# fgnt/pb_chime5

Hardware: AMD Instinct MI355X
Metric: utterance-seconds enhanced/sec/GPU (24ch, 20 EM iters) (higher is better)
Workload: dtype f64

## Files before the change

### pb_chime5_amd/csrc/cacgmm.hip

```cpp
#include <algorithm>
#include <cmath>
#include <cstdlib>

#include "gss_internal.h"
#include "dense_wave.h"
#include "jacobi.h"

namespace {

#ifndef GSS_CHOL_PRIO
#define GSS_CHOL_PRIO 1
#endif
#ifndef GSS_ESTEP_PRIO
#define GSS_ESTEP_PRIO 1
#endif
constexpr int EM_TILE = 64;
constexpr int EM_TS = EM_TILE + 1;

enum { MODE_FIRST = 0, MODE_EM = 1, MODE_PREDICT = 2 };

__device__ __forceinline__ void set_progress_priority(int done, int total) {
    const int q4 = 4 * done / total;
    if (q4 <= 0) __builtin_amdgcn_s_setprio(3);
    else if (q4 == 1) __builtin_amdgcn_s_setprio(2);
// ... 823 lines not shown
        cplx t[NS][CB];
#pragma unroll
        for (int s = 0; s < NS; ++s)
#pragma unroll
            for (int j = 0; j < CB; ++j)
                t[s][j] = (lane + 64 * s < NE && c + j < cnt) ? src[(int64_t)(c + j) * K * NE + 64 * s]
                                                              : c_make(0.0, 0.0);
#pragma unroll
        for (int s = 0; s < NS; ++s)
#pragma unroll
            for (int j = 0; j < CB; ++j) vals[s] = c_add(vals[s], t[s][j]);
    }
#pragma unroll
    for (int s = 0; s < NS; ++s) {
        if (lane + 64 * s < NE) {
            vals[s].x = ((double)D * vals[s].x) / den;
            vals[s].y = ((double)D * vals[s].y) / den;
        }
    }
#pragma unroll
    for (int s = 0; s < NS; ++s) {
        const int p = ts.d12[s];
        if (p >= 0 && (p >> 8) == (p & 255)) {
            vals[s].y = 0.0;
            tr += vals[s].x;
        }
    }
    return wave_sum(tr);
}

template <int NS = COV_SLOTS>
__device__ inline void store_covariance(const cplx (&vals)[COV_SLOTS], int D, double shift,
                                        bool full, cplx *A, int ld, int lane, const TriSlots &ts) {
#pragma unroll
    for (int s = 0; s < NS; ++s) {
        const int p = ts.d12[s];
        if (p >= 0) {
            const int d1 = p >> 8, d2 = p & 255;
            cplx v = vals[s];
            if (d1 == d2) v.x -= shift;
            A[d2 * ld + d1] = c_conj(v);
            if (full) A[d1 * ld + d2] = v;
        }
    }
}

#ifdef GSS_CHOL_TRACE
__device__ long long g_chol_phase[4096 * 10];
extern "C" int gss_debug_chol_phase(long long *host, int entries) {
    return (int)hipMemcpyFromSymbol(host, HIP_SYMBOL(g_chol_phase), sizeof(long long) * 10 * entries);
}
#define CHOL_STAMP(slot)                                                              \
    do {                                                                              \
        const int wg_ = blockIdx.y * gridDim.x + blockIdx.x;                          \
        if (threadIdx.x == 0 && wg_ < 4096) g_chol_phase[wg_ * 10 + (slot)] = clock64(); \
    } while (0)
#else
#define CHOL_STAMP(slot)
#endif

template <int NR>
__device__ __forceinline__ bool class_update_chol(const cplx (&vals)[COV_SLOTS], int D, int K,
                                                  double eig_floor, cplx *A, int lane,
                                                  cplx *__restrict__ Mq_fk,
                                                  double *__restrict__ logdet_fk,
                                                  const TriSlots &ts,
                                                  const int *__restrict__ tab_cm = nullptr) {
    constexpr int ld = 8 * NR + 1;
    constexpr int NS = cov_slots_for(NR);
    double *dinv = reinterpret_cast<double *>(A + D * ld);
    double nb2 = 0.0;
#pragma unroll
    for (int s = 0; s < NS; ++s) {
        const int p = ts.d12[s];
        if (p >= 0)
            nb2 += ((p >> 8) == (p & 255) ? 1.0 : 2.0) * (vals[s].x * vals[s].x + vals[s].y * vals[s].y);
    }
    nb2 = wave_sum(nb2);
    CHOL_STAMP(4);
    store_covariance<NS>(vals, D, 0.0, true, A, ld, lane, ts);
    wave_sync();
    const int tx = lane & 7, ty = lane >> 3;
    cplx reg[NR][NR];
#pragma unroll
    for (int a = 0; a < NR; ++a)
#pragma unroll
        for (int b = 0; b < NR; ++b) {
            const int i = ty + 8 * a, kk = tx + 8 * b;
            reg[a][b] = (kk >= i && kk < D) ? A[i * ld + kk] : c_make(0.0, 0.0);
        }
    wave_sync();
    CHOL_STAMP(5);
    if (!chol_inverse_sweep<8, NR, true>(reg, D, A, ld, dinv, tx, ty)) return false;
    CHOL_STAMP(6);
#if GSS_CHOL_PRIO
    __builtin_amdgcn_s_setprio(0);
#endif
    double ldv = 0.0;
    for (int i = lane; i < D; i += 64) ldv -= 2.0 * log(dinv[i]);
    ldv = wave_sum(ldv);
    CHOL_STAMP(7);
    double ni2 = 0.0;
    const int NE = tri_count(D);
#pragma unroll
    for (int s = 0; s < NS; ++s) {
        const int p = tab_cm ? (lane + 64 * s < NE ? tab_cm[lane + 64 * s] : -1) : ts.d12[s];
        if (p < 0) continue;
        const int d1 = p >> 8, d2 = p & 255;
// ... 54 lines not shown
#pragma unroll
        for (int s = 0; s < 4; ++s) {
            const int idx = lane + 64 * s, i = idx / m, j = idx - i * m;
            if (idx < m * m) {
                V[idx] = basis[idx];
                if (i <= j) {
                    A[i * m + j] = rot[s];
                    A[j * m + i] = c_conj(rot[s]);
                }
            }
        }
        wave_sync();
    }
    jacobi_eigh_wave(A, V, m, lane, 20, warm);
    if (basis != nullptr) {
        for (int idx = lane; idx < m * m; idx += 64) basis[idx] = V[idx];
        if (lane == 0) *basis_valid = 1;
    }
    double lmax = -INFINITY;
    for (int i = lane; i < D; i += 64) lmax = fmax(lmax, A[i * m + i].x);
    lmax = wave_max(lmax);
    double ldv = 0.0;
    for (int i = lane; i < D; i += 64) {
        double l = A[i * m + i].x / fmax(lmax, GSS_TINY);
        l = fmax(l, eig_floor);
        lam[i] = 1.0 / l;
        ldv += log(l);
    }
    ldv = wave_sum(ldv);
    wave_sync();
#pragma unroll
    for (int s = 0; s < COV_SLOTS; ++s) {
        const int p = ts.d12[s];
        if (p < 0) continue;
        const int e = lane + 64 * s, d1 = p >> 8, d2 = p & 255;
        cplx v = c_make(0.0, 0.0);
        for (int j = 0; j < D; ++j) {
            const cplx a = V[d1 * m + j], b = V[d2 * m + j];
            const double il = lam[j];
            v.x += il * (a.x * b.x + a.y * b.y);
            v.y += il * (a.y * b.x - a.x * b.y);
        }
        if (d1 == d2) {
            v.y = 0.0;
        } else {
            v.x *= 2.0;
            v.y *= 2.0;
        }
        Mq_fk[(int64_t)e * K] = v;
    }
    if (lane == 0) *logdet_fk = ldv;
}

template <int NR>
__global__ __launch_bounds__(64) void em_chol_kernel(const cplx *__restrict__ Bp,
                                                     const double *__restrict__ Sg, int nch,
                                                     int sg_nch, int D,
                                                     int K, int64_t T, double eig_floor,
                                                     int force_eigh, cplx *__restrict__ Mq,
                                                     double *__restrict__ logdet,
                                                     double *__restrict__ pi,
                                                     int *__restrict__ need_eigh,
                                                     const int *__restrict__ tri_tab,
                                                     MsegPlan plan,
                                                     const int *__restrict__ zero_tiles, int ntile) {
    extern __shared__ __attribute__((aligned(16))) char smem[];
    const int NE = tri_count(D);
    cplx *A = reinterpret_cast<cplx *>(smem);
    const int k = blockIdx.x, f = blockIdx.y, lane = threadIdx.x;
    const bool clamped = frequency_has_zero_frames(zero_tiles, ntile, f, lane);
    const int cnt = plan.S > 0 ? mseg_count(plan, f) : nch;

    CHOL_STAMP(0);
#if GSS_CHOL_PRIO
    __builtin_amdgcn_s_setprio(3);
#endif
    const TriSlots ts = tri_slots_tab(tri_tab, NE, lane);
    const double sg = sum_gamma(Sg, sg_nch, K, k, f, lane);
    const double den = fmax(sg, GSS_TINY);
    if (lane == 0) pi[f * K + k] = sg / (double)T;
    CHOL_STAMP(1);
    CHOL_STAMP(2);
    cplx vals[COV_SLOTS];
    const double tr = reduce_covariance<cov_slots_for(NR)>(Bp, nch, cnt, D, K, k, f, den, vals, lane, ts);
    CHOL_STAMP(3);
#if GSS_CHOL_PRIO
    __builtin_amdgcn_s_setprio(2);
#endif
    bool fast = !force_eigh && !clamped && tr > 0.0 && isfinite(tr);
    if (fast)
        fast = class_update_chol<NR>(vals, D, K, eig_floor, A, lane, Mq + (int64_t)f * NE * K + k,
                                     logdet + f * K + k, ts, tri_tab + NE);
    if (lane == 0) need_eigh[f * K + k] = fast ? 0 : 1;
    CHOL_STAMP(9);
}

__global__ __launch_bounds__(64) void em_eigh_kernel(const cplx *__restrict__ Bp,
                                                     const double *__restrict__ Sg, int nch,
                                                     int sg_nch, int D,
                                                     int K, double eig_floor,
                                                     const int *__restrict__ need_eigh,
                                                     cplx *__restrict__ Mq,
                                                     double *__restrict__ logdet,
                                                     const int *__restrict__ tri_tab,
                                                     MsegPlan plan) {
    const int k = blockIdx.x, f = blockIdx.y, lane = threadIdx.x;
    if (!need_eigh[f * K + k]) return;
    const int cnt = plan.S > 0 ? mseg_count(plan, f) : nch;
    extern __shared__ __attribute__((aligned(16))) char smem[];
    const int NE = tri_count(D);
    const double sg = sum_gamma(Sg, sg_nch, K, k, f, lane);
    const double den = fmax(sg, GSS_TINY);
    const TriSlots ts = tri_slots_tab(tri_tab, NE, lane);
    cplx vals[COV_SLOTS];
    reduce_covariance(Bp, nch, cnt, D, K, k, f, den, vals, lane, ts);
    class_update_eigh(vals, D, K, eig_floor, reinterpret_cast<cplx *>(smem), lane,
                      Mq + (int64_t)f * NE * K + k, logdet + f * K + k, ts);
}

__device__ __forceinline__ double row16_sum(double v) {
    double s = v + dpp_shifted<0x111, 0xf, 0xf>(v);
    s += dpp_shifted<0x112, 0xf, 0xf>(v);
    s += dpp_shifted<0x113, 0xf, 0xf>(v);
    s += dpp_shifted<0x114, 0xf, 0xe>(s);
    s += dpp_shifted<0x118, 0xf, 0xc>(s);
    return s;
}

constexpr int OC_FRAMES = 256;

#ifndef GSS_EM4_PRIO
#define GSS_EM4_PRIO 1
#endif
#ifdef GSS_EM4_TRACE
__device__ long long g_em4_phase[1024 * 6];
extern "C" int gss_debug_em4_phase(long long *host, int entries) {
    return (int)hipMemcpyFromSymbol(host, HIP_SYMBOL(g_em4_phase), sizeof(long long) * 6 * entries);
}
#define EM4_T(var) const long long var = __builtin_readcyclecounter()
#define EM4_ADD(slot, d) em4_acc[slot] += (d)
#else
#define EM4_T(var)
#define EM4_ADD(slot, d)
#endif

struct OnchipArgs {
    cplx *basis;
    const cplx *Yn;
    const uint8_t *act;
    int64_t act_stride, act_fstride;
    const double *init;
    int64_t init_stride, init_fstride;
    int64_t T;
    int F, iterations, iterations_post, force_eigh;
    int unmasked;
    const int *zero_tiles;
    int ntile;
    int cold_eigh;
    double eig_floor;
    double *gamma;
};

__device__ __forceinline__ bool class_update4_lane(const double (&b)[16], double eig_floor,
                                                   double (&m)[16], double &logdet) {
    constexpr int D = 4;
    cplx a[D][D];
    double nb2 = 0.0, tr = 0.0;
    {
        int off = 0;
#pragma unroll
// ... 627 lines not shown
};
EmStrides em_strides(const EmBlockPlan &p, int F, int64_t T, int D) {
    EmStrides s{0, 0, 0};
    for (int b : {0, p.nblocks - 1}) {
        const int Fb = em_block_size(p, F, b);
        int cf;
        const int nch = em_chunks(Fb, T, D, &cf);
        const int wpb = estep_waves_per_block(Fb, T);
        s.nch = std::max(s.nch, nch);
        s.reg_nch = std::max(s.reg_nch, wpb * (int)((T + 64 * wpb - 1) / (64 * wpb)));
    }
    s.bp_nch = std::max(s.nch, mstep_maxseg_limit());
    return s;
}

}

int psd_partials_run(gss_ctx *ctx, const cplx *Y, int F, int64_t T, int D, const double *W2,
                     int nch, int chunk_frames, cplx *part, int S) {
    const size_t lds = wcov_lds_layout(D, 2).total;
    const wcov_fn_t fn = D <= 4 ? wcov_kernel<2, false, false, false, 1>
                         : D <= 12 ? wcov_kernel<2, false, false, false, 3>
                         : D <= 24 ? wcov_kernel<2, false, false, false, 6> : wcov_kernel<2, false, false>;
    GSS_TRY(raise_lds_limit(ctx, fn, lds));
    hipLaunchKernelGGL(fn, dim3(xcd_grid(nch, F), S), dim3(256), lds,
                       ctx->stream, Y, W2, F, T, D, tri_count(D), nch, chunk_frames, part, 2, 0,
                       MsegPlan{});
    GSS_LAUNCH_CHECK(ctx, "wcov_kernel");
    return GSS_OK;
}

int psd3_partials_run(gss_ctx *ctx, const cplx *Y, int F, int64_t T, int D, const double *W3,
                      int nch, int chunk_frames, cplx *part) {
    const size_t lds = wcov_lds_layout(D, 3).total;
    const wcov_fn_t fn = D <= 4 ? wcov_kernel<3, false, false, false, 1>
                         : D <= 12 ? wcov_kernel<3, false, false, false, 3>
                         : D <= 24 ? wcov_kernel<3, false, false, false, 6> : wcov_kernel<3, false, false>;
    GSS_TRY(raise_lds_limit(ctx, fn, lds));
    hipLaunchKernelGGL(fn, dim3(xcd_grid(nch, F)), dim3(256), lds, ctx->stream, Y, W3, F, T, D,
                       tri_count(D), nch, chunk_frames, part, 3, 0, MsegPlan{});
    GSS_LAUNCH_CHECK(ctx, "wcov_kernel");
    return GSS_OK;
}

struct EmWork {
    cplx *Mq;
    double *logdet, *pi, *W;
    cplx *Bp;
    double *Sg_lds;
    cplx *Yn;
    double *Sg_reg;
    int *need_eigh;
    int *zero_tiles;
    int *tri_tab;
    cplx *basis;
};
static EmWork em_blocks(Workspace &ws, int F, int64_t T, int D, int K, const EmStrides &st,
                        bool onchip) {
    const size_t NE = tri_count(D);
    EmWork k;
    k.Mq = ws.take<cplx>((size_t)F * NE * K, "cacgmm Mq");
    k.logdet = ws.take<double>((size_t)F * K, "cacgmm logdet");
    k.pi = ws.take<double>((size_t)F * K, "cacgmm pi");
    k.W = ws.take<double>((size_t)F * K * T, "cacgmm W");
    k.Bp = ws.take<cplx>((size_t)F * st.bp_nch * K * NE, "cacgmm Bp");
    k.Sg_lds = ws.take<double>((size_t)F * st.nch * K, "cacgmm Sg");
    k.Yn = ws.take<cplx>((size_t)F * D * T, "cacgmm Yn");
    k.Sg_reg = ws.take<double>((size_t)F * st.reg_nch * K, "cacgmm Sg (register form)");
    k.need_eigh = ws.take<int>((size_t)F * K, "cacgmm need_eigh");
    k.zero_tiles = ws.take<int>((size_t)F * ((T + EM_TILE - 1) / EM_TILE), "cacgmm zero_tiles");
    k.tri_tab = ws.take<int>(2 * NE, "cacgmm tri_tab");
    k.basis = onchip ? ws.take<cplx>((size_t)F * K * 16, "cacgmm basis") : nullptr;
    return k;
}

size_t cacgmm_workspace_bytes(int F, int64_t T, int D, int K, bool one_block) {
    const EmBlockPlan bp = one_block ? EmBlockPlan{F, 1, 1} : em_block_plan(F, T, D, K);
    Workspace ws;
    em_blocks(ws, F, T, D, K, em_strides(bp, F, T, D), true);
    return ws.bytes + 4096;
}

namespace {
struct EmBlock {
    EmArgs a;
    int F, f0;
    cplx *Mq, *Yn;
    int *need_eigh, *zero_tiles;
    double *Sg_lds, *Sg_reg;
    int nch_lds, reg_nch, bp_nch, sg_nch;
    hipStream_t stream;
};
struct StreamRestore {
    gss_ctx *ctx;
    hipStream_t s;
    ~StreamRestore() { ctx->stream = s; }
};
}

int cacgmm_run(gss_ctx *ctx, const cplx *Y, int F, int64_t T, int D, const EmGuide &guide, int K,
               int iterations, int iterations_post, double *gamma) {
    EmSchedule s;
    s.iterations = iterations;
    s.model_iterations = std::max(iterations_post - 1, 0);
    s.model_masked = false;
    s.predict_masked = iterations_post == 0;
    s.gamma = gamma;
    s.onchip_allowed = true;
    return cacgmm_schedule_run(ctx, Y, F, T, D, guide, K, s);
}

int cacgmm_schedule_run(gss_ctx *ctx, const cplx *Y, int F, int64_t T, int D, const EmGuide &guide,
                        int K, const EmSchedule &s) {
    const int NE = tri_count(D);
    const int iterations = s.iterations;
    double *const gamma = s.gamma;
    const bool reg = estep_reg_supported(D, K) && !gss_variant_set("estep_lds");
    const bool onchip = s.onchip_allowed && D == 4 && K >= 2 && K <= 6 && reg && iterations > 0 &&
                        !gss_variant_set("em_unfused") && !s.shared_prior;
    const EmBlockPlan bplan =
        onchip || s.shared_prior ? EmBlockPlan{F, 1, 1} : em_block_plan(F, T, D, K);
    const EmStrides st = em_strides(bplan, F, T, D);

    GSS_REQUIRE(ctx, !s.shared_prior || (!s.import_model && !s.export_model && !s.loglik),
                GSS_ERR_INVALID, "cacgmm: a model with a shared prior cannot leave the call");
    Workspace ws(ctx);
    const EmWork k = em_blocks(ws, F, T, D, K, st, onchip);
    EmPriorWork pw{};
    if (s.shared_prior) {
        pw = cacgmm_prior_alloc(ws, F, T, K, !s.prior);
        if (s.prior) pw.prior = s.prior;
    }
    GSS_TRY(ws.status("cacgmm"));
    cplx *const Mq = k.Mq, *const Bp = k.Bp, *const Yn = k.Yn;
    double *const logdet = k.logdet, *const pi = k.pi, *const W = k.W;
    double *const Sg_lds = k.Sg_lds, *const Sg_reg = k.Sg_reg;
    int *const need_eigh = k.need_eigh, *const zero_tiles = k.zero_tiles, *const tri_tab = k.tri_tab;
    const int ntile = (int)((T + EM_TILE - 1) / EM_TILE);
    GSS_REQUIRE(ctx, em_estep_lds(D, K) <= 160 * 1024 &&
                         wcov_lds_layout(D, std::min(K, 8)).total <= 160 * 1024,
                GSS_ERR_UNSUPPORTED, "cacgmm: D=%d K=%d LDS", D, K);
    const bool has_mask = guide.mask != nullptr;
    const uint8_t *const act = has_mask ? guide.mask : reinterpret_cast<const uint8_t *>(Yn);
    const int64_t act_stride = has_mask ? guide.mask_k_stride : 0;
    const int64_t act_fstride = has_mask ? guide.mask_f_stride : 0;
    const int m = D + (D & 1);
    const size_t eigh_lds = (sizeof(cplx) * 2 * m * m + sizeof(double) * m + 15) / 16 * 16;
    const int force_eigh = gss_variant_set("force_eigh");
    if (!onchip) {
        hipLaunchKernelGGL(tri_table_kernel, dim3(1), dim3(256), 0, ctx->stream, D, tri_tab);
        GSS_LAUNCH_CHECK(ctx, "tri_table_kernel");
    }
    GSS_REQUIRE(ctx, !onchip || (!s.import_model && !s.export_model && !s.loglik), GSS_ERR_INVALID,
                "cacgmm: the one-launch kernel keeps its model on the chip");
    if (s.import_model) GSS_TRY(cacgmm_model_import(ctx, *s.import_model, F, K, D, Mq, logdet, pi));

    auto make_block = [&](int f0, int Fb, hipStream_t stream, EmBlock *blk) -> int {
        EmBlock &b = *blk;
        b = EmBlock{};
        b.F = Fb;
        b.f0 = f0;
        b.stream = stream;
        EmArgs &a = b.a;
        a.Y = Y + (int64_t)f0 * T * D;
        a.act = act + (int64_t)f0 * act_fstride;
        a.act_stride = act_stride;
        a.act_fstride = act_fstride;
        a.init = guide.init ? guide.init + (int64_t)f0 * guide.init_f_stride : nullptr;
        a.init_stride = guide.init_k_stride;
        a.init_fstride = guide.init_f_stride;
        a.T = T;
        a.F = Fb;
        a.D = D;
        a.NE = NE;
        a.nch = em_chunks(Fb, T, D, &a.chunk_frames);
        GSS_TRY(mstep_plan(ctx, Fb, T, D, K, &a.mseg));
        b.bp_nch = a.mseg.S > 0 ? a.mseg.maxseg : a.nch;
        b.nch_lds = a.nch;
        const int wpb = estep_waves_per_block(Fb, T);
        b.reg_nch = wpb * (int)((T + 64 * wpb - 1) / (64 * wpb));
        GSS_REQUIRE(ctx, b.bp_nch <= st.bp_nch && b.nch_lds <= st.nch && b.reg_nch <= st.reg_nch,
                    GSS_ERR_INVALID, "cacgmm: block strides");
        b.Mq = Mq + (int64_t)f0 * NE * K;
        a.logdet = logdet + (int64_t)f0 * K;
        a.pi = pi + (int64_t)f0 * K;
        a.W = W + (int64_t)f0 * K * T;
        a.Bp = Bp + (int64_t)f0 * st.bp_nch * K * NE;
        b.Sg_lds = Sg_lds + (int64_t)f0 * st.nch * K;
        b.Sg_reg = Sg_reg + (int64_t)f0 * st.reg_nch * K;
        a.Sg = b.Sg_lds;
        a.gamma = gamma ? gamma + (int64_t)f0 * K * T : nullptr;
        b.Yn = Yn + (int64_t)f0 * D * T;
        b.need_eigh = need_eigh + (int64_t)f0 * K;
        b.zero_tiles = zero_tiles + (int64_t)f0 * ntile;
        b.sg_nch = b.nch_lds;
        return GSS_OK;
    };
    auto prepare = [&](EmBlock &b) -> int {
        GSS_PROF(ctx, "em_prepare");
        const size_t plds = sizeof(cplx) * (size_t)D * EM_TS + sizeof(double) * 4 * EM_TILE;
        const auto prep = D <= 4 ? em_prepare_kernel<1> : D <= 12 ? em_prepare_kernel<3>
                          : D <= 24 ? em_prepare_kernel<6> : em_prepare_kernel<8>;
        hipLaunchKernelGGL(prep,
                           dim3(xcd_grid((int)((T + EM_TILE - 1) / EM_TILE), b.F)), dim3(256), plds,
                           ctx->stream, b.a.Y, b.F, T, D, b.Yn, b.zero_tiles);
        GSS_LAUNCH_CHECK(ctx, "em_prepare_kernel");
        return GSS_OK;
    };
    auto estep = [&](EmBlock &b, int mode) -> int {
        EmArgs &a = b.a;
        if (s.shared_prior) {
            a.Sg = pw.Sg;
            const EmPriorArgs p{b.Yn, b.Mq, a.logdet, pw.prior, a.act, a.act_stride, a.act_fstride,
                                a.init, a.init_stride, a.init_fstride, a.W, pw.G, pw.Sg, a.gamma,
                                T, b.F, D, a.masked, a.aff_eps};
            return cacgmm_prior_estep_run(ctx, p, K, mode == MODE_FIRST ? EM_PRIOR_FIRST
                                                     : mode == MODE_EM  ? EM_PRIOR_FIT
                                                                        : EM_PRIOR_PREDICT);
        }
        if (reg && mode != MODE_FIRST) {
            a.Sg = b.Sg_reg;
            switch (D) {
                case 24: return launch_estep_reg_k<24>(ctx, K, mode, a, b.Mq, b.Yn, b.F);
                case 20: return launch_estep_reg_k<20>(ctx, K, mode, a, b.Mq, b.Yn, b.F);
                case 12: return launch_estep_reg_k<12>(ctx, K, mode, a, b.Mq, b.Yn, b.F);
                case 10: return launch_estep_reg_k<10>(ctx, K, mode, a, b.Mq, b.Yn, b.F);
                default: return launch_estep_reg_k<4>(ctx, K, mode, a, b.Mq, b.Yn, b.F);
            }
        }
        a.Sg = b.Sg_lds;
        return launch_estep_k(ctx, K, mode, a, b.Mq, b.F);
    };
    auto eig = [&](EmBlock &b) -> int {
        EmArgs &a = b.a;
        {
            GSS_PROF(ctx, "em_chol");
            const int nr = (D + 7) / 8;
            const size_t lds = sizeof(cplx) * (size_t)D * (8 * nr + 1) + sizeof(double) * D;
            auto kern = nr <= 1 ? em_chol_kernel<1> : nr == 2 ? em_chol_kernel<2>
                        : nr == 3 ? em_chol_kernel<3> : em_chol_kernel<4>;
            hipLaunchKernelGGL(kern, dim3(K, b.F), dim3(64), lds, ctx->stream, a.Bp, a.Sg, b.bp_nch,
                               b.sg_nch, D, K, T, 1e-10, force_eigh, b.Mq,
                               const_cast<double *>(a.logdet), const_cast<double *>(a.pi),
                               b.need_eigh, tri_tab, a.mseg, b.zero_tiles, ntile);
            GSS_LAUNCH_CHECK(ctx, "em_chol_kernel");
        }
        {
            GSS_PROF(ctx, "em_eigh");
            hipLaunchKernelGGL(em_eigh_kernel, dim3(K, b.F), dim3(64), eigh_lds, ctx->stream, a.Bp,
                               a.Sg, b.bp_nch, b.sg_nch, D, K, 1e-10, b.need_eigh, b.Mq,
                               const_cast<double *>(a.logdet), tri_tab, a.mseg);
            GSS_LAUNCH_CHECK(ctx, "em_eigh_kernel");
        }
        return GSS_OK;
    };

    if (onchip) {
        EmBlock b;
        GSS_TRY(make_block(0, F, ctx->stream, &b));
        GSS_TRY(prepare(b));
        OnchipArgs o{};
        o.basis = k.basis;
        o.Yn = Yn;
        o.act = act;
        o.act_stride = act_stride;
        o.act_fstride = act_fstride;
        o.init = guide.init;
        o.init_stride = guide.init_k_stride;
        o.init_fstride = guide.init_f_stride;
        o.unmasked = has_mask ? 0 : 1;
        o.T = T;
        o.F = F;
        o.iterations = iterations;
        o.iterations_post = s.predict_masked ? 0 : s.model_iterations + 1;
        o.force_eigh = force_eigh;
        o.zero_tiles = b.zero_tiles;
        o.ntile = ntile;
        o.cold_eigh = gss_variant_set("em4_cold_eigh");
        o.eig_floor = 1e-10;
        o.gamma = gamma;
        switch (K) {
            case 2: return launch_onchip4<2>(ctx, o);
            case 3: return launch_onchip4<3>(ctx, o);
            case 4: return launch_onchip4<4>(ctx, o);
            case 5: return launch_onchip4<5>(ctx, o);
            default: return launch_onchip4<6>(ctx, o);
        }
    }

    auto em_iteration = [&](EmBlock &b, bool first) -> int {
        GSS_TRY(estep(b, first ? MODE_FIRST : MODE_EM));
        b.sg_nch = s.shared_prior ? ntile : (reg && !first) ? b.reg_nch : b.nch_lds;
        if (s.shared_prior) {
            const bool one_table = guide.init ? guide.init_f_stride == 0 : guide.mask_f_stride == 0;
            GSS_TRY(cacgmm_prior_update_run(ctx, pw, first && one_table ? 1 : F, K, T));
        }
        GSS_TRY(launch_mstep_k(ctx, K, b.a, b.Yn, b.F));
        return eig(b);
    };

// ... 56 lines not shown
```

### pb_chime5_amd/csrc/gss_api.hip

```cpp
#include <cmath>
#include <cstdarg>
#include <cstdlib>
#include <cstring>
#include <mutex>

#include "gss_internal.h"

#define GSS_ENTER(ctx)                                   \
    if (!(ctx)) return GSS_ERR_INVALID;                  \
    GSS_HIP_CHECK((ctx), hipSetDevice((ctx)->device))
#define GSS_ENTER_VARIANTS(ctx) \
    GSS_ENTER(ctx);             \
    GSS_TRY(variant_refresh(ctx))
static int variant_refresh(gss_ctx *ctx);

#define GSS_STATUS_REF_CHANNEL 0
#define GSS_STATUS_WPE_ZERO_PIVOTS 2

static std::mutex g_error_lock;

int gss_fail(gss_ctx *ctx, int code, const char *fmt, ...) {
    char buf[1024];
    va_list ap;
    va_start(ap, fmt);
    vsnprintf(buf, sizeof(buf), fmt, ap);
    va_end(ap);
    if (ctx) {
        std::lock_guard<std::mutex> guard(g_error_lock);
        ctx->error = buf;
    }
    return code;
}

static thread_local std::string g_create_error;

namespace {
const char *const kVariantKeys[] = {
    "corr_ts", "corr_nw", "corr_blocked", "corr_p_tiles", "chol_diag_unfolded", "apply_ph",
    "apply_generic", "prof_detail", "corr_stg8", "corr_ksplit", "apply_gglobal", "wpe_halves",
    "em_wgs", "estep_wpb", "estep_lds", "mstep_prefetch_d", "mstep_tiled", "mstep_plan_min_d",
    "mstep_chunked", "mstep_slots", "force_eigh", "em_unfused", "em_l3_mb", "em_l3_fit_mb",
    "em_streams", "mstep_maxseg", "em4_cold_eigh", "mstep_generic",
    "wpe_online_mem"};
struct VariantTable {
    std::mutex lock;
    std::string text;
    bool parsed = false;
    std::map<std::string, int> values;
};
VariantTable &variant_table() {
    static VariantTable t;
    return t;
}
}

static int variant_refresh(gss_ctx *ctx) {
    const char *env = getenv("GSS_VARIANT");
    VariantTable &t = variant_table();
    std::lock_guard<std::mutex> guard(t.lock);
    if (t.parsed && t.text == (env ? env : "")) return GSS_OK;
    t.text = env ? env : "";
    t.parsed = true;
    t.values.clear();
    std::string unknown;
    size_t pos = 0;
    while (pos < t.text.size()) {
        size_t end = t.text.find_first_of(", ", pos);
        if (end == std::string::npos) end = t.text.size();
        const std::string tok = t.text.substr(pos, end - pos);
        pos = end + 1;
        if (tok.empty()) continue;
        const size_t eq = tok.find('=');
        const std::string name = tok.substr(0, eq);
        bool known = false;
        for (const char *k : kVariantKeys) known = known || name == k;
        if (!known) {
            unknown = name;
            continue;
        }
        t.values[name] = eq == std::string::npos ? 1 : atoi(tok.c_str() + eq + 1);
    }
    if (!unknown.empty()) {
        t.values.clear();
        t.parsed = false;
        return gss_fail(ctx, GSS_ERR_INVALID, "GSS_VARIANT names no switch '%s'", unknown.c_str());
    }
    return GSS_OK;
}

int gss_variant(const char *key, int dflt) {
    VariantTable &t = variant_table();
    std::lock_guard<std::mutex> guard(t.lock);
    const auto it = t.values.find(key);
    return it == t.values.end() ? dflt : it->second;
}
// ... 45 lines not shown
        g_create_error = "device_id out of range";
        return GSS_ERR_INVALID;
    }
    e = hipSetDevice(device_id);
    if (e != hipSuccess) {
        g_create_error = hipGetErrorString(e);
        return GSS_ERR_HIP;
    }
    gss_ctx *ctx = new gss_ctx();
    ctx->device = device_id;
    e = hipStreamCreateWithFlags(&ctx->own_stream, hipStreamNonBlocking);
    if (e != hipSuccess) {
        g_create_error = hipGetErrorString(e);
        delete ctx;
        return GSS_ERR_HIP;
    }
    ctx->stream = ctx->own_stream;
    e = hipHostMalloc(reinterpret_cast<void **>(&ctx->status_host), GSS_STATUS_BYTES,
                      hipHostMallocMapped);
    if (e == hipSuccess)
        e = hipHostGetDevicePointer(reinterpret_cast<void **>(&ctx->status_dev), ctx->status_host, 0);
    if (e != hipSuccess) {
        g_create_error = hipGetErrorString(e);
        (void)hipStreamDestroy(ctx->own_stream);
        delete ctx;
        return GSS_ERR_HIP;
    }
    ctx->status_host[GSS_STATUS_REF_CHANNEL] = INT32_MIN;
    ctx->status_host[GSS_STATUS_WPE_ZERO_PIVOTS] = 0;
    ctx->status_host[GSS_STATUS_SEGMENT_FALLBACKS] = 0;
    ctx->status_host[GSS_STATUS_LCMV_INTERFERER] = -1;
    ctx->status_host[GSS_STATUS_LCMV_FALLBACKS] = 0;
    ctx->status_host[GSS_STATUS_WPD_ZERO_PIVOTS] = 0;
    ctx->status_host[GSS_STATUS_ALIGN_MOVED] = 0;
    *out = ctx;
    return GSS_OK;
}

static void free_tables(gss_ctx *ctx) {
    if (ctx->win_analysis) (void)hipFree(ctx->win_analysis);
    if (ctx->win_synthesis) (void)hipFree(ctx->win_synthesis);
    if (ctx->twiddle) (void)hipFree(ctx->twiddle);
    ctx->win_analysis = ctx->win_synthesis = nullptr;
    ctx->twiddle = nullptr;
}

extern "C" int gss_destroy(gss_ctx *ctx) {
    if (!ctx) return GSS_OK;
    (void)hipSetDevice(ctx->device);
    (void)hipStreamSynchronize(ctx->stream);
    free_tables(ctx);
    if (ctx->arena) (void)hipFree(ctx->arena);
    if (ctx->wpe_tiles) (void)hipFree(ctx->wpe_tiles);
    if (ctx->status_host) (void)hipHostFree(ctx->status_host);
    for (auto &p : ctx->prof_pending) {
        (void)hipEventDestroy(p.start);
        (void)hipEventDestroy(p.stop);
    }
    for (auto ev : ctx->event_pool) (void)hipEventDestroy(ev);
    if (ctx->ev_fork) (void)hipEventDestroy(ctx->ev_fork);
    if (ctx->ev_join) (void)hipEventDestroy(ctx->ev_join);
    if (ctx->aux_stream) {
        (void)hipStreamSynchronize(ctx->aux_stream);
        (void)hipStreamDestroy(ctx->aux_stream);
    }
    if (ctx->own_stream) (void)hipStreamDestroy(ctx->own_stream);
    delete ctx;
    return GSS_OK;
}

int aux_stream_ready(gss_ctx *ctx) {
    if (!ctx->aux_stream)
        GSS_HIP_CHECK(ctx, hipStreamCreateWithFlags(&ctx->aux_stream, hipStreamNonBlocking));
    if (!ctx->ev_fork) GSS_HIP_CHECK(ctx, hipEventCreateWithFlags(&ctx->ev_fork, hipEventDisableTiming));
    if (!ctx->ev_join) GSS_HIP_CHECK(ctx, hipEventCreateWithFlags(&ctx->ev_join, hipEventDisableTiming));
    return GSS_OK;
}

extern "C" int gss_set_stream(gss_ctx *ctx, void *hip_stream) {
    GSS_ENTER(ctx);
    GSS_HIP_CHECK(ctx, hipStreamSynchronize(ctx->stream));
    ctx->stream = hip_stream ? reinterpret_cast<hipStream_t>(hip_stream) : ctx->own_stream;
    return GSS_OK;
}

extern "C" int gss_set_utterances_in_flight(gss_ctx *ctx, int n) {
    if (!ctx) return GSS_ERR_INVALID;
    GSS_REQUIRE(ctx, n >= 0, GSS_ERR_INVALID, "gss_set_utterances_in_flight: n=%d", n);
    ctx->utterances_in_flight = n;
    return GSS_OK;
}

extern "C" int gss_synchronize(gss_ctx *ctx) {
    if (!ctx) return GSS_ERR_INVALID;
    GSS_HIP_CHECK(ctx, hipSetDevice(ctx->device));
    GSS_HIP_CHECK(ctx, hipStreamSynchronize(ctx->stream));
    return GSS_OK;
}

extern "C" int gss_dev_malloc(gss_ctx *ctx, size_t bytes, void **dev_ptr) {
    if (!ctx || !dev_ptr) return GSS_ERR_INVALID;
    GSS_HIP_CHECK(ctx, hipSetDevice(ctx->device));
    *dev_ptr = nullptr;
    if (bytes == 0) bytes = 16;
    hipError_t e = hipMalloc(dev_ptr, bytes);
    if (e != hipSuccess)
// ... 154 lines not shown
            if (ctx->debug_violations++ == 0) {
                char text[256];
                snprintf(text, sizeof(text),
                         "the guard headroom of the workspace debug mode (%zu bytes) is used up at "
                         "block %d%s%s: no sizing bug of the call",
                         kDebugHeadroom, ctx->debug_blocks, tag ? " " : "", tag ? tag : "");
                ctx->debug_first = text;
            }
            return nullptr;
        }
        ctx->debug_guards.push_back({ctx->debug_blocks++, off, bytes, phys + bytes,
                                     guard_end - (phys + bytes), tag, false});
        ctx->debug_phys = guard_end;
        ctx->arena_off = off + bytes;
        if (ctx->arena_off > ctx->arena_peak) ctx->arena_peak = ctx->arena_off;
        return ctx->arena + phys;
    }
    if (off + bytes > ctx->arena_size) return nullptr;
    ctx->arena_off = off + bytes;
    if (ctx->arena_off > ctx->arena_peak) ctx->arena_peak = ctx->arena_off;
    return ctx->arena + off;
}

int arena_release_debug(gss_ctx *ctx, size_t mark) {
    GSS_TRY(debug_sync(ctx));
    while (!ctx->debug_guards.empty() &&
           ctx->debug_guards.back().logical_off + ctx->debug_guards.back().bytes > mark) {
        GSS_TRY(debug_check_guard(ctx, ctx->debug_guards.back()));
        ctx->debug_guards.pop_back();
    }
    ctx->arena_off = mark;
    ctx->debug_phys = ctx->debug_guards.empty()
                          ? 0
                          : ctx->debug_guards.back().guard_off + ctx->debug_guards.back().guard_bytes;
    GSS_HIP_CHECK(ctx, hipMemsetAsync(ctx->arena + ctx->debug_phys, ctx->debug_pattern,
                                      ctx->arena_size - ctx->debug_phys, ctx->stream));
    return GSS_OK;
}

extern "C" int gss_debug_workspace(gss_ctx *ctx, int pattern) {
    GSS_ENTER(ctx);
    GSS_REQUIRE(ctx, pattern >= -1 && pattern <= 255, GSS_ERR_INVALID,
                "gss_debug_workspace: pattern=%d (a byte, or -1 for off)", pattern);
    GSS_TRY(debug_sync(ctx));
    ctx->debug_pattern = pattern;
    ctx->debug_guards.clear();
    ctx->debug_blocks = 0;
    ctx->debug_phys = 0;
    ctx->debug_logical_size = 0;
    ctx->debug_violations = 0;
    ctx->debug_first.clear();
    ctx->arena_off = 0;
    ctx->wpe_tiles_key[0] = ctx->wpe_tiles_key[1] = ctx->wpe_tiles_key[2] = ctx->wpe_tiles_key[3] = -1;
    return GSS_OK;
}

extern "C" int gss_debug_workspace_report(gss_ctx *ctx, int64_t *violations, char *buf, int len,
                                          int guard_index, void **guard_dev) {
    GSS_ENTER(ctx);
    if (guard_dev) *guard_dev = nullptr;
    if (violations) *violations = 0;
    if (buf && len > 0) buf[0] = 0;
    GSS_REQUIRE(ctx, ctx->debug_pattern >= 0, GSS_ERR_INVALID,
                "gss_debug_workspace_report: the workspace debug mode is off");
    GSS_TRY(debug_check_live_guards(ctx));
    if (violations) *violations = ctx->debug_violations;
    if (buf && len > 0) snprintf(buf, (size_t)len, "%s", ctx->debug_first.c_str());
    if (guard_dev && guard_index >= 0 && (size_t)guard_index < ctx->debug_guards.size())
        *guard_dev = ctx->arena + ctx->debug_guards[guard_index].guard_off;
    return GSS_OK;
}

extern "C" size_t gss_workspace_bytes(gss_ctx *ctx) { return ctx ? ctx->arena_peak : 0; }

ProfScope::ProfScope(gss_ctx *c, const char *name) : ctx(c), active(c->profiling) {
    if (active && !c->prof_filter.empty() && c->prof_filter != name) active = false;
    if (!active) return;
    e.name = name;
    auto get = [&]() {
        hipEvent_t ev;
        if (!ctx->event_pool.empty()) {
            ev = ctx->event_pool.back();
            ctx->event_pool.pop_back();
        } else {
            (void)hipEventCreate(&ev);
        }
        return ev;
    };
    e.start = get();
    e.stop = get();
    (void)hipEventRecord(e.start, ctx->stream);
}

ProfScope::~ProfScope() {
    if (!active) return;
    (void)hipEventRecord(e.stop, ctx->stream);
    ctx->prof_pending.push_back(e);
}

static void prof_drain(gss_ctx *ctx) {
    (void)hipStreamSynchronize(ctx->stream);
    for (auto &p : ctx->prof_pending) {
        float ms = 0.f;
        if (hipEventElapsedTime(&ms, p.start, p.stop) == hipSuccess) {
            auto &acc = ctx->prof_acc[p.name];
            acc.first += 1;
// ... 1865 lines not shown
```

### pb_chime5_amd/csrc/gss_internal.h

```cpp
#pragma once
#include <hip/hip_runtime.h>

#include <cstdint>
#include <cstdio>
#include <map>
#include <string>
#include <vector>

#include "../../include/gss_hip.h"

typedef double2 cplx;

int gss_variant(const char *key, int dflt);
inline bool gss_variant_set(const char *key) { return gss_variant(key, 0) != 0; }

#if (defined(GSS_CORR_TRACE) || defined(GSS_WCOV_TRACE) || defined(GSS_EM4_TRACE) || \
     defined(GSS_CHOL_TRACE)) && !defined(GSS_EXPERIMENT_BUILD)
#error "trace instrumentation needs -DGSS_EXPERIMENT_BUILD=1 (tools/build_variant.sh)"
#endif

#define GSS_TINY 2.2250738585072014e-308

__device__ __forceinline__ cplx c_make(double r, double i) { return make_double2(r, i); }
__device__ __forceinline__ cplx c_add(cplx a, cplx b) { return make_double2(a.x + b.x, a.y + b.y); }
// ... 76 lines not shown
static inline unsigned xcd_grid(int nsub, int F) { return (unsigned)(nsub * ((F + 7) / 8 * 8)); }

__host__ __device__ __forceinline__ int tri_index(int d1, int d2, int D) {
    return d1 * D - (d1 * (d1 - 1)) / 2 + (d2 - d1);
}
__host__ __device__ __forceinline__ int tri_count(int D) { return D * (D + 1) / 2; }

struct ProfEntry {
    std::string name;
    hipEvent_t start, stop;
};

struct gss_ctx {
    int device = 0;
    hipStream_t own_stream = nullptr;
    hipStream_t stream = nullptr;
    hipStream_t aux_stream = nullptr;
    hipEvent_t ev_fork = nullptr, ev_join = nullptr;
    int utterances_in_flight = 0;
    std::string error;

    char *arena = nullptr;
    size_t arena_size = 0;
    size_t arena_off = 0;
    size_t arena_peak = 0;

    struct DebugGuard {
        int block;
        size_t logical_off, bytes;
        size_t guard_off, guard_bytes;
        const char *tag;
        bool reported;
    };
    int debug_pattern = -1;
    size_t debug_phys = 0;
    size_t debug_logical_size = 0;
    int debug_blocks = 0;
    std::vector<DebugGuard> debug_guards;
    int64_t debug_violations = 0;
    std::string debug_first;

    int stft_size = 0, stft_shift = 0;
    double *win_analysis = nullptr;
    double *win_synthesis = nullptr;
    cplx *twiddle = nullptr;

    int32_t *status_host = nullptr;
    int32_t *status_dev = nullptr;
    int last_targets = 0;
    int last_selected = 0;

    void *wpe_tiles = nullptr;
    int wpe_tiles_key[4] = {-1, -1, -1, -1};

    bool profiling = false;
    std::vector<ProfEntry> prof_pending;
    std::vector<hipEvent_t> event_pool;
    std::map<std::string, std::pair<long, double>> prof_acc;
    std::string prof_filter;
};

#define GSS_STATUS_SEGMENT_FALLBACKS 3
#define GSS_STATUS_LCMV_INTERFERER 4
#define GSS_STATUS_LCMV_FALLBACKS 5
#define GSS_STATUS_WPD_ZERO_PIVOTS 6
#define GSS_STATUS_ALIGN_MOVED 7
#define GSS_STATUS_MVDR_ONLINE_FALLBACKS 8
#define GSS_STATUS_CACGMM_ONLINE_FALLBACKS 9
#define GSS_STATUS_CACGMM_ONLINE_BAD_MODEL 10
#define GSS_STATUS_TARGETS 16
#define GSS_STATUS_CHANNELS 40
#define GSS_STATUS_BYTES (4 * (GSS_STATUS_CHANNELS + GSS_MAX_CHANNELS))
static_assert(GSS_STATUS_TARGETS + GSS_MAX_CLASSES + 1 <= GSS_STATUS_CHANNELS, "status words overlap");

int gss_fail(gss_ctx *ctx, int code, const char *fmt, ...);

#define GSS_HIP_CHECK(ctx, expr)                                                   \
    do {                                                                           \
        hipError_t _e = (expr);                                                    \
        if (_e != hipSuccess)                                                      \
            return gss_fail((ctx), GSS_ERR_HIP, "%s failed: %s (%s:%d)", #expr,    \
                            hipGetErrorString(_e), __FILE__, __LINE__);            \
    } while (0)

#define GSS_REQUIRE(ctx, cond, code, ...)                      \
    do {                                                       \
        if (!(cond)) return gss_fail((ctx), (code), __VA_ARGS__); \
    } while (0)

#define GSS_TRY(expr)              \
    do {                           \
        int _s = (expr);           \
        if (_s != GSS_OK) return _s; \
    } while (0)

int arena_reserve(gss_ctx *ctx, size_t bytes);
void arena_reset(gss_ctx *ctx);
void *arena_alloc(gss_ctx *ctx, size_t bytes, const char *tag);
int arena_release_debug(gss_ctx *ctx, size_t mark);
static inline int arena_release(gss_ctx *ctx, size_t mark) {
    if (ctx->debug_pattern >= 0) return arena_release_debug(ctx, mark);
    ctx->arena_off = mark;
    return GSS_OK;
}
static inline size_t align_up(size_t v, size_t a = 256) { return (v + a - 1) / a * a; }

// ... 230 lines not shown
```

Baseline: 1095.

## Fold eigh fallback into chol kernel, pack two waves per block, cache tri table

The Cholesky M-step kernel now packs two matrices per 128-thread workgroup, one per wave, over a flattened grid. Flagged matrices get the eigendecomposition fallback inside the same kernel after a block barrier, which removes the separate em_eigh launch per EM iteration by default. The triangle index table moves into the context and is rebuilt only when D changes, so the per-run tri_table_kernel launch goes away. The cost is a serialized fallback loop with __syncthreads and larger LDS per block, which may lower occupancy.

```diff
diff --git a/pb_chime5_amd/csrc/cacgmm.hip b/pb_chime5_amd/csrc/cacgmm.hip
--- a/pb_chime5_amd/csrc/cacgmm.hip
+++ b/pb_chime5_amd/csrc/cacgmm.hip
@@ -899,8 +899,8 @@
 }
 #define CHOL_STAMP(slot)                                                              \
     do {                                                                              \
-        const int wg_ = blockIdx.y * gridDim.x + blockIdx.x;                          \
-        if (threadIdx.x == 0 && wg_ < 4096) g_chol_phase[wg_ * 10 + (slot)] = clock64(); \
+        const int wg_ = blockIdx.x * (blockDim.x >> 6) + (threadIdx.x >> 6);    \
+        if ((threadIdx.x & 63) == 0 && wg_ < 4096) g_chol_phase[wg_ * 10 + (slot)] = clock64(); \
     } while (0)
 #else
 #define CHOL_STAMP(slot)
@@ -1061,47 +1061,97 @@
     if (lane == 0) *logdet_fk = ldv;
 }
 
+__device__ __forceinline__ void class_redo_eigh(const cplx *__restrict__ Bp,
+                                                const double *__restrict__ Sg, int nch, int sg_nch,
+                                                int D, int K, int k, int f, double eig_floor,
+                                                cplx *__restrict__ Mq, double *__restrict__ logdet,
+                                                const int *__restrict__ tri_tab, const MsegPlan &plan,
+                                                char *smem, int lane) {
+    const int cnt = plan.S > 0 ? mseg_count(plan, f) : nch;
+    const int NE = tri_count(D);
+    const double sg = sum_gamma(Sg, sg_nch, K, k, f, lane);
+    const double den = fmax(sg, GSS_TINY);
+    const TriSlots ts = tri_slots_tab(tri_tab, NE, lane);
+    cplx vals[COV_SLOTS];
+    reduce_covariance(Bp, nch, cnt, D, K, k, f, den, vals, lane, ts);
+    class_update_eigh(vals, D, K, eig_floor, reinterpret_cast<cplx *>(smem), lane,
+                      Mq + (int64_t)f * NE * K + k, logdet + f * K + k, ts);
+}
+
+__host__ __device__ constexpr size_t em_chol_wave_lds(int D, int NR) {
+    return (sizeof(cplx) * (size_t)D * (8 * NR + 1) + sizeof(double) * D + 15) / 16 * 16;
+}
+
 template <int NR>
-__global__ __launch_bounds__(64) void em_chol_kernel(const cplx *__restrict__ Bp,
-                                                     const double *__restrict__ Sg, int nch,
-                                                     int sg_nch, int D,
-                                                     int K, int64_t T, double eig_floor,
-                                                     int force_eigh, cplx *__restrict__ Mq,
-                                                     double *__restrict__ logdet,
-                                                     double *__restrict__ pi,
-                                                     int *__restrict__ need_eigh,
-                                                     const int *__restrict__ tri_tab,
-                                                     MsegPlan plan,
-                                                     const int *__restrict__ zero_tiles, int ntile) {
+__global__ __launch_bounds__(128) void em_chol_kernel(const cplx *__restrict__ Bp,
+                                                      const double *__restrict__ Sg, int nch,
+                                                      int sg_nch, int D,
+                                                      int K, int64_t T, double eig_floor,
+                                                      int force_eigh, cplx *__restrict__ Mq,
+                                                      double *__restrict__ logdet,
+                                                      double *__restrict__ pi,
+                                                      int *__restrict__ need_eigh,
+                                                      const int *__restrict__ tri_tab,
+                                                      MsegPlan plan,
+                                                      const int *__restrict__ zero_tiles, int ntile,
+                                                      int nmat, int redo_eigh, int flag_off) {
     extern __shared__ __attribute__((aligned(16))) char smem[];
     const int NE = tri_count(D);
-    cplx *A = reinterpret_cast<cplx *>(smem);
-    const int k = blockIdx.x, f = blockIdx.y, lane = threadIdx.x;
-    const bool clamped = frequency_has_zero_frames(zero_tiles, ntile, f, lane);
-    const int cnt = plan.S > 0 ? mseg_count(plan, f) : nch;
-
-    CHOL_STAMP(0);
+    const int wave = __builtin_amdgcn_readfirstlane(threadIdx.x >> 6), lane = threadIdx.x & 63;
+    const int i = blockIdx.x * (blockDim.x >> 6) + wave;
+    const bool live = i < nmat;
+    const int f = live ? i / K : 0, k = live ? i - f * K : 0;
+    bool fast = true;
+    if (live) {
+        cplx *A = reinterpret_cast<cplx *>(smem + wave * em_chol_wave_lds(D, NR));
+        const bool clamped = frequency_has_zero_frames(zero_tiles, ntile, f, lane);
+        const int cnt = plan.S > 0 ? mseg_count(plan, f) : nch;
+
+        CHOL_STAMP(0);
 #if GSS_CHOL_PRIO
-    __builtin_amdgcn_s_setprio(3);
+        __builtin_amdgcn_s_setprio(3);
 #endif
-    const TriSlots ts = tri_slots_tab(tri_tab, NE, lane);
-    const double sg = sum_gamma(Sg, sg_nch, K, k, f, lane);
-    const double den = fmax(sg, GSS_TINY);
-    if (lane == 0) pi[f * K + k] = sg / (double)T;
-    CHOL_STAMP(1);
-    CHOL_STAMP(2);
-    cplx vals[COV_SLOTS];
-    const double tr = reduce_covariance<cov_slots_for(NR)>(Bp, nch, cnt, D, K, k, f, den, vals, lane, ts);
-    CHOL_STAMP(3);
+        const TriSlots ts = tri_slots_tab(tri_tab, NE, lane);
+        const double sg = sum_gamma(Sg, sg_nch, K, k, f, lane);
+        const double den = fmax(sg, GSS_TINY);
+        if (lane == 0) pi[f * K + k] = sg / (double)T;
+        CHOL_STAMP(1);
+        CHOL_STAMP(2);
+        cplx vals[COV_SLOTS];
+        const double tr = reduce_covariance<cov_slots_for(NR)>(Bp, nch, cnt, D, K, k, f, den, vals, lane, ts);
+        CHOL_STAMP(3);
 #if GSS_CHOL_PRIO
-    __builtin_amdgcn_s_setprio(2);
+        __builtin_amdgcn_s_setprio(2);
 #endif
-    bool fast = !force_eigh && !clamped && tr > 0.0 && isfinite(tr);
-    if (fast)
-        fast = class_update_chol<NR>(vals, D, K, eig_floor, A, lane, Mq + (int64_t)f * NE * K + k,
-                                     logdet + f * K + k, ts, tri_tab + NE);
-    if (lane == 0) need_eigh[f * K + k] = fast ? 0 : 1;
-    CHOL_STAMP(9);
+        fast = !force_eigh && !clamped && tr > 0.0 && isfinite(tr);
+        if (fast)
+            fast = class_update_chol<NR>(vals, D, K, eig_floor, A, lane, Mq + (int64_t)f * NE * K + k,
+                                         logdet + f * K + k, ts, tri_tab + NE);
+        if (lane == 0) need_eigh[f * K + k] = fast ? 0 : 1;
+        CHOL_STAMP(9);
+    }
+    if (!redo_eigh) return;
+#if GSS_CHOL_PRIO
+    __builtin_amdgcn_s_setprio(0);
+#endif
+    int *flags = reinterpret_cast<int *>(smem + flag_off);
+    if (lane == 0) flags[wave] = fast ? 0 : 1;
+    __syncthreads();
+    const int nwave = blockDim.x >> 6;
+    int flagged[2];
+    flagged[0] = __builtin_amdgcn_readfirstlane(flags[0]);
+    flagged[1] = nwave > 1 ? __builtin_amdgcn_readfirstlane(flags[1]) : 0;
+#pragma nounroll
+    for (int w = 0; w < nwave; ++w) {
+        if (!flagged[w]) continue;
+        if (wave == w) {
+            int lane2 = lane;
+            asm volatile("" : "+v"(lane2));
+            class_redo_eigh(Bp, Sg, nch, sg_nch, D, K, k, f, eig_floor, Mq, logdet, tri_tab, plan,
+                            smem, lane2);
+        }
+        __syncthreads();
+    }
 }
 
 __global__ __launch_bounds__(64) void em_eigh_kernel(const cplx *__restrict__ Bp,
@@ -1115,16 +1165,8 @@
                                                      MsegPlan plan) {
     const int k = blockIdx.x, f = blockIdx.y, lane = threadIdx.x;
     if (!need_eigh[f * K + k]) return;
-    const int cnt = plan.S > 0 ? mseg_count(plan, f) : nch;
     extern __shared__ __attribute__((aligned(16))) char smem[];
-    const int NE = tri_count(D);
-    const double sg = sum_gamma(Sg, sg_nch, K, k, f, lane);
-    const double den = fmax(sg, GSS_TINY);
-    const TriSlots ts = tri_slots_tab(tri_tab, NE, lane);
-    cplx vals[COV_SLOTS];
-    reduce_covariance(Bp, nch, cnt, D, K, k, f, den, vals, lane, ts);
-    class_update_eigh(vals, D, K, eig_floor, reinterpret_cast<cplx *>(smem), lane,
-                      Mq + (int64_t)f * NE * K + k, logdet + f * K + k, ts);
+    class_redo_eigh(Bp, Sg, nch, sg_nch, D, K, k, f, eig_floor, Mq, logdet, tri_tab, plan, smem, lane);
 }
 
 __device__ __forceinline__ double row16_sum(double v) {
@@ -1858,7 +1900,6 @@
     double *Sg_reg;
     int *need_eigh;
     int *zero_tiles;
-    int *tri_tab;
     cplx *basis;
 };
 static EmWork em_blocks(Workspace &ws, int F, int64_t T, int D, int K, const EmStrides &st,
@@ -1875,7 +1916,6 @@
     k.Sg_reg = ws.take<double>((size_t)F * st.reg_nch * K, "cacgmm Sg (register form)");
     k.need_eigh = ws.take<int>((size_t)F * K, "cacgmm need_eigh");
     k.zero_tiles = ws.take<int>((size_t)F * ((T + EM_TILE - 1) / EM_TILE), "cacgmm zero_tiles");
-    k.tri_tab = ws.take<int>(2 * NE, "cacgmm tri_tab");
     k.basis = onchip ? ws.take<cplx>((size_t)F * K * 16, "cacgmm basis") : nullptr;
     return k;
 }
@@ -1904,6 +1944,24 @@
 };
 }
 
+static int em_tri_table(gss_ctx *ctx, int D, const int **tab) {
+    GSS_REQUIRE(ctx, D >= 1 && D <= GSS_MAX_CHANNELS, GSS_ERR_UNSUPPORTED, "cacgmm: D=%d", D);
+    if (!ctx->tri_tab) {
+        GSS_HIP_CHECK(ctx, hipMalloc(&ctx->tri_tab, sizeof(int) * 2 * tri_count(GSS_MAX_CHANNELS)));
+        ctx->tri_tab_d = -1;
+    }
+    if (ctx->tri_tab_d != D) {
+        if (ctx->debug_pattern >= 0)
+            GSS_HIP_CHECK(ctx, hipMemsetAsync(ctx->tri_tab, ctx->debug_pattern,
+                                              sizeof(int) * 2 * tri_count(GSS_MAX_CHANNELS), ctx->stream));
+        hipLaunchKernelGGL(tri_table_kernel, dim3(1), dim3(256), 0, ctx->stream, D, ctx->tri_tab);
+        GSS_LAUNCH_CHECK(ctx, "tri_table_kernel");
+        ctx->tri_tab_d = D;
+    }
+    *tab = ctx->tri_tab;
+    return GSS_OK;
+}
+
 int cacgmm_run(gss_ctx *ctx, const cplx *Y, int F, int64_t T, int D, const EmGuide &guide, int K,
                int iterations, int iterations_post, double *gamma) {
     EmSchedule s;
@@ -1941,7 +1999,8 @@
     cplx *const Mq = k.Mq, *const Bp = k.Bp, *const Yn = k.Yn;
     double *const logdet = k.logdet, *const pi = k.pi, *const W = k.W;
     double *const Sg_lds = k.Sg_lds, *const Sg_reg = k.Sg_reg;
-    int *const need_eigh = k.need_eigh, *const zero_tiles = k.zero_tiles, *const tri_tab = k.tri_tab;
+    int *const need_eigh = k.need_eigh, *const zero_tiles = k.zero_tiles;
+    const int *tri_tab = nullptr;
     const int ntile = (int)((T + EM_TILE - 1) / EM_TILE);
     GSS_REQUIRE(ctx, em_estep_lds(D, K) <= 160 * 1024 &&
                          wcov_lds_layout(D, std::min(K, 8)).total <= 160 * 1024,
@@ -1953,10 +2012,7 @@
     const int m = D + (D & 1);
     const size_t eigh_lds = (sizeof(cplx) * 2 * m * m + sizeof(double) * m + 15) / 16 * 16;
     const int force_eigh = gss_variant_set("force_eigh");
-    if (!onchip) {
-        hipLaunchKernelGGL(tri_table_kernel, dim3(1), dim3(256), 0, ctx->stream, D, tri_tab);
-        GSS_LAUNCH_CHECK(ctx, "tri_table_kernel");
-    }
+    if (!onchip) GSS_TRY(em_tri_table(ctx, D, &tri_tab));
     GSS_REQUIRE(ctx, !onchip || (!s.import_model && !s.export_model && !s.loglik), GSS_ERR_INVALID,
                 "cacgmm: the one-launch kernel keeps its model on the chip");
     if (s.import_model) GSS_TRY(cacgmm_model_import(ctx, *s.import_model, F, K, D, Mq, logdet, pi));
@@ -2037,21 +2093,27 @@
         a.Sg = b.Sg_lds;
         return launch_estep_k(ctx, K, mode, a, b.Mq, b.F);
     };
+    const bool eigh_launch = gss_variant_set("em_eigh_launch");
     auto eig = [&](EmBlock &b) -> int {
         EmArgs &a = b.a;
+        const int nr = std::min((D + 7) / 8, 4);
+        const size_t wave_lds = em_chol_wave_lds(D, nr);
+        const int nmat = K * b.F;
         {
             GSS_PROF(ctx, "em_chol");
-            const int nr = (D + 7) / 8;
-            const size_t lds = sizeof(cplx) * (size_t)D * (8 * nr + 1) + sizeof(double) * D;
             auto kern = nr <= 1 ? em_chol_kernel<1> : nr == 2 ? em_chol_kernel<2>
                         : nr == 3 ? em_chol_kernel<3> : em_chol_kernel<4>;
-            hipLaunchKernelGGL(kern, dim3(K, b.F), dim3(64), lds, ctx->stream, a.Bp, a.Sg, b.bp_nch,
-                               b.sg_nch, D, K, T, 1e-10, force_eigh, b.Mq,
-                               const_cast<double *>(a.logdet), const_cast<double *>(a.pi),
-                               b.need_eigh, tri_tab, a.mseg, b.zero_tiles, ntile);
+            const int waves = eigh_launch ? 1 : 2;
+            const size_t flag_off = std::max(2 * wave_lds, eigh_lds);
+            const size_t lds = eigh_launch ? wave_lds : flag_off + 16;
+            hipLaunchKernelGGL(kern, dim3((nmat + waves - 1) / waves), dim3(64 * waves), lds,
+                               ctx->stream, a.Bp, a.Sg, b.bp_nch, b.sg_nch, D, K, T, 1e-10,
+                               force_eigh, b.Mq, const_cast<double *>(a.logdet),
+                               const_cast<double *>(a.pi), b.need_eigh, tri_tab, a.mseg,
+                               b.zero_tiles, ntile, nmat, eigh_launch ? 0 : 1, (int)flag_off);
             GSS_LAUNCH_CHECK(ctx, "em_chol_kernel");
         }
-        {
+        if (eigh_launch) {
             GSS_PROF(ctx, "em_eigh");
             hipLaunchKernelGGL(em_eigh_kernel, dim3(K, b.F), dim3(64), eigh_lds, ctx->stream, a.Bp,
                                a.Sg, b.bp_nch, b.sg_nch, D, K, 1e-10, b.need_eigh, b.Mq,
diff --git a/pb_chime5_amd/csrc/gss_api.hip b/pb_chime5_amd/csrc/gss_api.hip
--- a/pb_chime5_amd/csrc/gss_api.hip
+++ b/pb_chime5_amd/csrc/gss_api.hip
@@ -40,7 +40,7 @@
     "apply_generic", "prof_detail", "corr_stg8", "corr_ksplit", "apply_gglobal", "wpe_halves",
     "em_wgs", "estep_wpb", "estep_lds", "mstep_prefetch_d", "mstep_tiled", "mstep_plan_min_d",
     "mstep_chunked", "mstep_slots", "force_eigh", "em_unfused", "em_l3_mb", "em_l3_fit_mb",
-    "em_streams", "mstep_maxseg", "em4_cold_eigh", "mstep_generic",
+    "em_streams", "mstep_maxseg", "em4_cold_eigh", "mstep_generic", "em_eigh_launch",
     "wpe_online_mem"};
 struct VariantTable {
     std::mutex lock;
@@ -192,6 +192,7 @@
     free_tables(ctx);
     if (ctx->arena) (void)hipFree(ctx->arena);
     if (ctx->wpe_tiles) (void)hipFree(ctx->wpe_tiles);
+    if (ctx->tri_tab) (void)hipFree(ctx->tri_tab);
     if (ctx->status_host) (void)hipHostFree(ctx->status_host);
     for (auto &p : ctx->prof_pending) {
         (void)hipEventDestroy(p.start);
@@ -452,6 +453,7 @@
     ctx->debug_first.clear();
     ctx->arena_off = 0;
     ctx->wpe_tiles_key[0] = ctx->wpe_tiles_key[1] = ctx->wpe_tiles_key[2] = ctx->wpe_tiles_key[3] = -1;
+    ctx->tri_tab_d = -1;
     return GSS_OK;
 }
 
diff --git a/pb_chime5_amd/csrc/gss_internal.h b/pb_chime5_amd/csrc/gss_internal.h
--- a/pb_chime5_amd/csrc/gss_internal.h
+++ b/pb_chime5_amd/csrc/gss_internal.h
@@ -152,6 +152,9 @@
 
     void *wpe_tiles = nullptr;
     int wpe_tiles_key[4] = {-1, -1, -1, -1};
+
+    int *tri_tab = nullptr;
+    int tri_tab_d = -1;
 
     bool profiling = false;
     std::vector<ProfEntry> prof_pending;
```

New measurement: 1097 (median of 6 runs). About the same (+0.1%).
